# p-mc-grath/DMMFODS

Measured on AMD Instinct MI355X. Metric: training images/sec at 1280x1920 RGB+LiDAR, higher is better.
Workload: dtype f16; 1 GPU; C2 d121 early-fusion 6ch b4 1280x1920; key=c2, per_gpu_batch=4, global_batch=4, height=1280, width=1920, storage_dtype=fp16, accumulate=fp32, parallelism=dp1, weights=random-init (reference init, seed 123)

## Files before the change

dmmfods_amd/_lib.py:

```python
import ctypes as C
import os

_HERE = os.path.dirname(os.path.abspath(__file__))
LIB_PATH = os.environ.get("DMM_LIB_PATH") or os.path.join(_HERE, "libdmmfods_hip.so")

DMM_F32, DMM_F16, DMM_BF16 = 0, 1, 2
LOSS_BCE, LOSS_FOCAL = 0, 1
T_CONV, T_CONVT, T_BN_WEIGHT, T_BN_BIAS, T_BN_MEAN, T_BN_VAR, T_BN_TRACKED = range(7)
ERR_INVALID, ERR_SHAPE, ERR_HIP, ERR_STATE, ERR_NO_DEVICE = -1, -2, -3, -4, -5


class ModelDesc(C.Structure):
    _fields_ = [
        ("growth_rate", C.c_int32), ("num_blocks", C.c_int32), ("block_config", C.c_int32 * 8),
        ("num_init_features", C.c_int32), ("bn_size", C.c_int32), ("num_classes", C.c_int32),
        ("concat_before_block_num", C.c_int32), ("stream_1_in_channels", C.c_int32),
        ("stream_2_in_channels", C.c_int32), ("batch", C.c_int32), ("height", C.c_int32), ("width", C.c_int32),
        ("dtype", C.c_int32), ("loss_scale", C.c_float), ("bn_momentum", C.c_float), ("bn_eps", C.c_float),
        ("iou_threshold", C.c_float), ("use_mfma", C.c_int32),
    ]


class ConvDesc(C.Structure):
    _fields_ = [(n, C.c_int32) for n in (
# ... 119 lines not shown
    L.dmm_plan_set_encoder_frozen.argtypes = [vp, C.c_int]
    L.dmm_adam_table_bytes.argtypes = [C.c_int, i64]
    L.dmm_adam_table_bytes.restype = sz
    L.dmm_adam_table_init.argtypes = [vp, C.POINTER(AdamSegment), C.c_int, i64, C.c_int, vp]
    L.dmm_adam_step_segmented.argtypes = [vp, vp, vp, vp, i64, vp, C.c_int, C.POINTER(AdamClass), C.c_int, i64, f32, vp]
    L.dmm_adam_step_guarded_segmented.argtypes = [vp, vp, vp, vp, i64, vp, C.c_int, C.POINTER(AdamClass), C.c_int, f32, f32, f32, i32,
                                                  vp, vp, vp]
    L.dmm_adam_step_segmented_ema.argtypes = L.dmm_adam_step_segmented.argtypes + [C.POINTER(AdamEma)]
    L.dmm_adam_step_guarded_segmented_ema.argtypes = L.dmm_adam_step_guarded_segmented.argtypes + [C.POINTER(AdamEma)]
    L.dmm_grad_sumsq.argtypes = [vp, i64, i64, C.c_int, vp, vp]
    L.dmm_plan_set_dynamic_loss_scale.argtypes = [vp, vp]
    L.dmm_plan_set_grad_accumulate.argtypes = [vp, C.c_int]
    L.dmm_conv_scratch_bytes.argtypes = [C.POINTER(ConvDesc)]
    L.dmm_conv_scratch_bytes.restype = sz
    L.dmm_conv_forward.argtypes = [C.POINTER(ConvDesc), vp, vp, vp, vp, vp, vp, vp, vp]
    L.dmm_conv_logits.argtypes = [C.POINTER(ConvDesc), vp, vp, vp, vp, vp, vp, vp]
    L.dmm_conv_wgrad.argtypes = [C.POINTER(ConvDesc), vp, vp, vp, vp, vp, vp, vp]
    L.dmm_conv_dgrad.argtypes = [C.POINTER(ConvDesc), vp, vp, vp, vp, vp, vp, vp, vp, vp]
    L.dmm_conv_wgrad_ex.argtypes = [C.POINTER(ConvDesc), vp, vp, vp, vp, vp, vp, vp, C.c_int, vp, vp, vp]
    L.dmm_conv_dgrad_ex.argtypes = [C.POINTER(ConvDesc), vp, vp, vp, vp, vp, vp, vp, vp, vp, C.c_int, vp, vp, vp]
    L.dmm_conv1x1_backward_fused.argtypes = [C.POINTER(ConvDesc), vp, vp, vp, vp, vp, vp, vp, vp, vp, C.c_int, vp, vp, vp, vp]
    L.dmm_conv5_wgrad_stats.argtypes = [C.POINTER(ConvDesc), vp, vp, vp, vp, vp, vp, vp, vp, vp]
    L.dmm_plan_wgrad_batch_counts.argtypes = [vp, C.POINTER(C.c_longlong * 4)]
    L.dmm_conv_wgrad_grouped.argtypes = [C.POINTER(ConvDesc), C.c_int, vp, vp, vp, vp, vp, vp, vp, vp, vp, C.c_int, C.POINTER(C.c_int), vp]
    L.dmm_bw1_reduce_grouped.argtypes = [C.c_int, vp, vp, C.POINTER(C.c_int), C.POINTER(C.c_int), C.POINTER(C.c_int), C.c_int,
                                         C.POINTER(C.c_int), vp]
    _lib = L
    return L


EXPORTS = [
    "dmm_last_error", "dmm_version", "dmm_set_option", "dmm_plan_create", "dmm_plan_destroy", "dmm_plan_num_tensors",
    "dmm_plan_tensor_info", "dmm_plan_num_params", "dmm_plan_num_buffer_elems", "dmm_plan_workspace_bytes",
    "dmm_plan_forward_flops", "dmm_plan_bind", "dmm_plan_forward", "dmm_plan_loss_backward", "dmm_plan_backward",
    "dmm_plan_loss_metrics", "dmm_plan_num_graph_replays", "dmm_plan_set_loss", "dmm_loss_forward", "dmm_plan_num_grad_buckets", "dmm_plan_grad_bucket",
    "dmm_plan_grad_bucket_wait", "dmm_plan_profile_begin", "dmm_plan_profile_filter", "dmm_plan_profile_num_ops", "dmm_plan_profile_op",
    "dmm_plan_profile_collect", "dmm_adam_step", "dmm_conv_scratch_bytes", "dmm_conv_forward", "dmm_conv_logits", "dmm_conv_wgrad",
    "dmm_conv_dgrad", "dmm_conv_wgrad_ex", "dmm_conv_dgrad_ex", "dmm_conv1x1_backward_fused", "dmm_conv5_wgrad_stats", "dmm_last_impl", "dmm_impl_name", "dmm_impl_mask",
    "dmm_grad_guard_scratch_bytes", "dmm_guard_state_init", "dmm_adam_step_guarded", "dmm_grad_sumsq", "dmm_plan_set_dynamic_loss_scale",
    "dmm_plan_set_grad_accumulate", "dmm_plan_set_encoder_frozen",
    "dmm_adam_table_bytes", "dmm_adam_table_init", "dmm_adam_step_segmented", "dmm_adam_step_guarded_segmented",
    "dmm_adam_step_segmented_ema", "dmm_adam_step_guarded_segmented_ema",
    "dmm_plan_wgrad_batch_counts", "dmm_conv_wgrad_grouped", "dmm_bw1_reduce_grouped",
    "dmm_logit_hist_elems", "dmm_logit_hist", "dmm_augment_batch",
]
HIST_MAX_THRESHOLDS = 255


def check(rc):
    if rc == 0:
        return
    msg = lib().dmm_last_error().decode(errors="replace")
    if rc == ERR_SHAPE:
        raise ValueError(msg)
    if rc == ERR_INVALID and "fusion" in msg:
        raise AttributeError(msg)
    if rc == ERR_INVALID:
        raise ValueError(msg)
    raise DmmError(f"dmm status {rc}: {msg}")
# ... 17 lines not shown
```

dmmfods_amd/csrc/capi.cpp:

```cpp
#include <algorithm>
#include <atomic>
#include <cmath>
#include <cstdio>
#include <cstdlib>
#include <cstring>
#include <stdexcept>
#include <mutex>
#include <string>
#include <utility>
#include <vector>
#include <unistd.h>

#include "dispatch.h"
#include "plan.h"

using namespace dmm;

void plan_build_tables(dmm_plan* p);
void plan_bind(dmm_plan* p, void* ws);
void plan_size(dmm_plan* p);

static thread_local std::string g_err;
static int fail(int code, const std::string& msg) {
  g_err = msg;
// ... 210 lines not shown
    case OP_IGEMM: return launch_igemm(o.c, dt, o.epi, mfma, st, o.impl);
    case OP_WGRAD:
      if (o.impl == IMPL_WG3 && o.w.M > 0) { ++p->batch_counts[0]; ++p->batch_counts[1]; }
      return launch_wgrad(o.w, dt, mfma, st, o.impl);
    case OP_BW1: return launch_bw1(o.b1, dt, st);
    case OP_BW1RED:
      { Bw1RedGroup one; if (bw1_reduce_group_add(one, o.b1) && one.n > 0) { ++p->batch_counts[2]; ++p->batch_counts[3]; } }
      return launch_bw1_reduce(o.b1, st);
    case OP_RAWFIN: return launch_wg5_rawfin(o.rf, st);
    case OP_FIN64: return launch_wg5_fin64(o.f64, st);
    case OP_JOIN: if (o.epi == 1) lanes.join_pack(); else lanes.join_side(); return hipSuccess;
    case OP_BNFIN: return launch_bn_finalize(o.bf, st);
    case OP_BNBWD:
      if (accumulate) { BnBwdFinalizeArgs bb = o.bb; bb.accumulate = 1; return launch_bn_bwd_finalize(bb, st); }
      return launch_bn_bwd_finalize(o.bb, st);
    case OP_POOL: return launch_maxpool_fwd(o.mp, dt, st);
    case OP_POOLBWD: return launch_maxpool_bwd(o.mpb, dt, st);
    case OP_BCE: return launch_bce_metrics(o.bce, dt, st);
    case OP_PACK: return launch_pack(o.pk.descs, o.pk.prefix, o.pk.ndesc, o.pk.total_rows, dt, st, o.pk.tdescs, o.pk.tiles, o.pk.nt1, o.pk.nt9);
    case OP_APPLYCORR: return launch_apply_corr(o.ac, dt, st);
    case OP_UNPACK: return launch_unpack(o.pk.descs, o.pk.prefix, o.pk.ndesc, o.pk.total_rows, dt, o.pk.grad_scale, st, o.pk.tdescs, o.pk.tiles, o.pk.nt1, o.pk.nt9, accumulate);
    default: known = false; return hipSuccess;
  }
}

int launch_checked(dmm_plan* p, const Op& o, size_t i, hipStream_t st, Lanes& lanes, std::string& why) {
  const bool fam_check = (o.kind == OP_IGEMM || o.kind == OP_WGRAD) && o.impl != IMPL_AUTO;
  const unsigned mask_before = g_impl_mask;
  if (fam_check) g_impl_mask = 0;
  bool known = true;
  const hipError_t e = launch_record(p, o, st, lanes, known);
// ... 310 lines not shown
  if (B < 1 || NC < 1 || H < 1 || W < 1) return fail(DMM_ERR_INVALID, who + "B, NC, H and W must be >= 1");
  if ((long long)B * NC > 65535) return fail(DMM_ERR_INVALID, who + "B * NC must be <= 65535");
  if ((long long)H * W >= (1ll << 31)) return fail(DMM_ERR_INVALID, who + "H * W must be < 2^31");
  if (nthr < 1 || nthr > DMM_HIST_MAX_THRESHOLDS) return fail(DMM_ERR_INVALID, who + "nthr must be in [1, " + std::to_string(DMM_HIST_MAX_THRESHOLDS) + "]");
  for (int k = 0; k < nthr; ++k)
    if (!std::isfinite(thresholds[k])) return fail(DMM_ERR_INVALID, who + "thresholds[" + std::to_string(k) + "] is NaN or infinite");
  for (int k = 1; k < nthr; ++k)
    if (!(thresholds[k] > thresholds[k - 1])) return fail(DMM_ERR_INVALID, who + "thresholds must be strictly ascending (at index " + std::to_string(k) + ")");
  if (std::isnan(gt_threshold)) return fail(DMM_ERR_INVALID, who + "gt_threshold is NaN");
  LogitHistArgs a;
  memset(&a, 0, sizeof(a));
  a.logits = logits; a.target = target; a.counts = (unsigned long long*)counts;
  a.B = B; a.NC = NC; a.H = H; a.W = W; a.K = nthr; a.gt = gt_threshold;
  for (int k = 0; k < nthr; ++k) a.thr[k] = thresholds[k];
  HIPCHK(launch_logit_hist(a, accumulate, (hipStream_t)stream));
  return DMM_OK;
}

int dmm_augment_batch(const dmm_aug_tensor* tensors, int ntensors, const dmm_aug_sample* samples, int B, int Hs, int Ws, int Ho, int Wo,
                      const float* fill, void* stream) {
  const std::string who = "dmm_augment_batch: ";
  if (!tensors || !samples) return fail(DMM_ERR_INVALID, who + "null argument");
  if (ntensors < 1 || ntensors > DMM_AUG_MAX_TENSORS) return fail(DMM_ERR_INVALID, who + "ntensors must be in [1, " + std::to_string(DMM_AUG_MAX_TENSORS) + "]");
  if (B < 1 || Hs < 1 || Ws < 1 || Ho < 1 || Wo < 1) return fail(DMM_ERR_INVALID, who + "B, Hs, Ws, Ho and Wo must be >= 1");
  const long long splane = (long long)Hs * Ws, dplane = (long long)Ho * Wo;
  if (splane >= (1ll << 31)) return fail(DMM_ERR_INVALID, who + "Hs * Ws must be < 2^31");
  if (dplane >= (1ll << 31)) return fail(DMM_ERR_INVALID, who + "Ho * Wo must be < 2^31");
  int nch = 0;
  for (int t = 0; t < ntensors; ++t) {
    const dmm_aug_tensor& T = tensors[t];
// ... 1019 lines not shown
```

dmmfods_amd/csrc/igemm.hip:

```cpp
#include <cstdlib>
#include <type_traits>

#ifndef IGEMM_FOLD_EPI
#define IGEMM_FOLD_EPI -1
#endif
#ifndef IGEMM_FOLD_BN
#define IGEMM_FOLD_BN 0
#endif
#ifndef IGEMM_FOLD_LIN
#define IGEMM_FOLD_LIN -1
#endif
#ifndef IGEMM_FOLD_PRO
#define IGEMM_FOLD_PRO -2
#endif
#ifndef IGEMM_F32_FOLD
#define IGEMM_F32_FOLD 0
#endif
#include "common.h"
#include "dispatch.h"
#include "gather.h"
#include "isa.h"

namespace dmm {

// ... 502 lines not shown
    }
    const int nsub = a.pool2 ? 4 : 1;
    const float wgt = a.pool2 ? 0.25f : 1.f;
    for (int row = rr; row < BM && !prefetched; row += RPP) {
      const int pix = rowpix[row];
      if (pix < 0 || !colvalid) continue;
      float av[SLOT];
#pragma unroll
      for (int i = 0; i < SLOT; i += 4) {
        const f32x4 t4 = *(const f32x4*)(Cs + row * SM::STAGE_PITCH_F + cv * SLOT + i);
        av[i] = t4[0]; av[i + 1] = t4[1]; av[i + 2] = t4[2]; av[i + 3] = t4[3];
      }
      for (int sub = 0; sub < nsub; ++sub) {
        const size_t p = (size_t)pix + (sub >> 1) * a.Wout + (sub & 1);
        float xf[SLOT], gf[SLOT];
        vec_to_f32<T>(*(const V*)(bx + p * a.ldbx + n), xf);
        if (a.accumulate && g != nullptr) vec_to_f32<T>(*(const V*)(g + p * a.ldo + n), gf);
#pragma unroll
        for (int i = 0; i < SLOT; ++i) {
          const float dz = (fmaf(xf[i], sc[i], sh[i]) > 0.f) ? av[i] * wgt : 0.f;
          s1[i] += dz;
          s2[i] = fmaf(dz, (xf[i] - mu[i]) * is[i], s2[i]);
          gf[i] = (a.accumulate ? gf[i] : 0.f) + sc[i] * dz;
        }
        if (g != nullptr) *(V*)(g + p * a.ldo + n) = f32_to_vec<T>(gf);
      }
    }
  }

  constexpr bool F32FOLD = IGEMM_F32_FOLD && (IGEMM_FOLD_EPI < 0 || EPI == IGEMM_FOLD_EPI) && (IGEMM_FOLD_BN == 0 || BN == IGEMM_FOLD_BN) &&
                           (IGEMM_FOLD_LIN < 0 || (int)LIN == IGEMM_FOLD_LIN) && (IGEMM_FOLD_PRO < -1 || PRO == IGEMM_FOLD_PRO);
  if constexpr ((sizeof(T) == 4 || !MFMA) && !F32FOLD) {
// ... 152 lines not shown
```

dmmfods_amd/csrc/plan.cpp:

```cpp
#include "plan.h"

#include <algorithm>
#include <cmath>
#include <cstdio>
#include <cstdlib>
#include <cstring>
#include <map>
#include <stdexcept>

namespace dmm {

static unsigned tw1(int mt) { return 0xffffff00u | (unsigned)mt; }

std::vector<Tap> taps_conv(int R, int S, int pad) {
  std::vector<Tap> t;
  for (int ky = 0; ky < R; ++ky)
    for (int kx = 0; kx < S; ++kx) t.push_back({ky - pad, kx - pad, tw1(ky * S + kx)});
  return t;
}
std::vector<Tap> taps_conv_dgrad(int R, int S, int pad) {
  std::vector<Tap> t;
  for (int ky = 0; ky < R; ++ky)
    for (int kx = 0; kx < S; ++kx) t.push_back({pad - ky, pad - kx, tw1(ky * S + kx)});
  return t;
// ... 236 lines not shown
struct ConvRec {
  std::string wname;
  bool transposed;
  int N, Kin, R, S, pad;
  int B, Ho, Wo;
  int nseg;
  SegRec seg[2];
  int obuf, och0, ostride;
  int epi;
  bool stats;
  std::vector<PhaseRec> phases;
  int dpack[2];
  bool wgrad_transposed;
  bool shared_master;
  double flops_ref;
};
struct PoolRec { int y0buf, bn, obuf, och0; uint8_t* argmax; int C; };
struct Rec { int type; int idx; };
struct BucketRec {
  int64_t off = 0, n = 0;
  int convs_left = 0, bns_left = 0;
  int first_desc = 0, ndesc = 0, rows = 0;
  int tile0 = 0, nt1 = 0, nt9 = 0;
  int last_main = -1, last_side = -1;
};

enum LaunchRole { ROLE_STORE, ROLE_BNBWD, ROLE_LOGITS, ROLE_WGRAD , ROLE_WGRAD_T  };
const char* launch_class(int impl, LaunchRole role) {
  static const struct { LaunchRole role; int impl; const char* cls; } table[] = {
      {ROLE_STORE, IMPL_CONV3, "conv3.store"}, {ROLE_STORE, IMPL_CVP, "cvp.store"},     {ROLE_STORE, IMPL_CF, "cf.store"},
// ... 206 lines not shown
    std::string s = w;
    const char* cuts[] = {"features.", "stream_2_features.", "decoder.", "dec_out_to_heat_maps.", ".weight", "denseblock", "denselayer", "Transposed_Convolution"};
    const char* reps[] = {"f.", "s2.", "d.", "h.", "", "b", "l", "TC"};
    for (int i = 0; i < 8; ++i) {
      size_t p;
      while ((p = s.find(cuts[i])) != std::string::npos) s.replace(p, strlen(cuts[i]), reps[i]);
    }
    return s;
  }
  double conv_flops(const ConvRec& c, size_t nphases) const {
    if (c.flops_ref > 0) return c.flops_ref / (double)nphases;
    const double px = (double)c.B * c.Ho * c.Wo * (c.seg[0].mode == G_POOL2 ? 4.0 : 1.0);
    const double f = c.transposed ? 2.0 * px * c.N * c.Kin * 9.0 : 2.0 * px * c.N * c.Kin * c.R * c.S;
    return f / (double)nphases;
  }
  double src_bytes(const ConvRec& c) const {
    double b = 0;
    for (int s = 0; s < c.nseg; ++s) {
      const Buf& sb = bufs[c.seg[s].buf];
      b += (double)sb.B * sb.H * sb.W * c.seg[s].C * esz;
    }
    return b;
  }
  double out_bytes(const ConvRec& c) const {
    const Buf& ob = bufs[c.obuf];
    return (double)ob.B * ob.H * ob.W * rup(c.N, 8) * (c.epi == EPI_LOGITS ? 4 : esz);
  }
  double w_bytes(const ConvRec& c) const { return (double)c.N * c.Kin * c.R * c.S * esz; }
  const uint8_t* xat(int buf, int ch) const { return bufs[buf].x + (size_t)ch * esz; }
  uint8_t* gat(int buf, int ch) const { return bufs[buf].g ? bufs[buf].g + (size_t)ch * esz : nullptr; }

  void emit_bn_finalize(int bn) {
    Bn& b = bns[bn];
    for (auto& rg : b.ranges) {
// ... 40 lines not shown
      const Op& po = (*ops)[first + ph];
      copy_phase(merged, po, ph);
      merged.flops += po.flops; merged.bytes += po.bytes;
    }
    if (!accept(merged)) return;
    ops->resize(first);
    ops->push_back(merged);
  }
  static void copy_fwd_phase(ConvArgs& m, const ConvArgs& po, int ph, int ntaps0) {
    m.nphase = 4;
    for (int t = 0; t < 4; ++t) m.ph_taps0[ph][t] = po.seg[0].taps[t < ntaps0 ? t : 0];
    m.ph_wpack[ph] = po.wpack;
    m.ph_py[ph] = (signed char)po.py; m.ph_px[ph] = (signed char)po.px;
  }

  void emit_conv_fwd(ConvRec& c) {
    for (int s = 0; s < c.nseg; ++s) {
      const int bn = c.seg[s].bn;
      if (bn < 0 || (s == 1 && bn == c.seg[0].bn)) continue;
      emit_bn_finalize(bn);
    }
    const Buf& ob = bufs[c.obuf];
    const bool mfma = d.use_mfma != 0;
    for (auto& ph : c.phases) {
      Op& o = push(OP_IGEMM);
      o.epi = c.epi;
      ConvArgs& a = o.c;
      a.nseg = c.nseg;
      for (int s = 0; s < c.nseg; ++s) fill_fwd_seg(a.seg[s], c.seg[s], (s == 1 && !ph.taps1.empty()) ? ph.taps1 : ph.taps);
      a.B = c.B; a.Ho = c.Ho; a.Wo = c.Wo; a.M = c.B * c.Ho * c.Wo;
      const PackDesc& pd = P.packs[ph.pack];
      a.wpack = pd.dst;
      a.N = c.N; a.Npad = pd.Npad;
      a.out = (void*)xat(c.obuf, c.och0);
      a.ldo = ob.ld; a.Hout = ob.H; a.Wout = ob.W;
      a.ostride = c.ostride; a.py = ph.py; a.px = ph.px;
      if (c.stats && ob.ssum) { a.stat_sum = ob.ssum + c.och0; a.stat_sq = ob.ssq + c.och0; a.stat_stride = ob.ld; }
      const double np = (double)c.phases.size();
      o.impl = igemm_pick(a, dtype, c.epi, mfma, deny);
      tag(o, ncls(o.impl, c.epi == EPI_LOGITS ? ROLE_LOGITS : ROLE_STORE, pd.Npad), short_name(c.wname), conv_flops(c, c.phases.size()),
          (src_bytes(c) + out_bytes(c)) / np + w_bytes(c) / np);
      if (c.epi == EPI_LOGITS) {
        if (training) P.logits_op_train = (int)ops->size() - 1; else P.logits_op_eval = (int)ops->size() - 1;
      }
// ... 152 lines not shown
    if (st.eff_compact != nullptr && o.impl == IMPL_WG3 && !leaf_scope) {
      st.wg3_op = o;
      ops->pop_back();
      st.wg3_held = true;
    } else if (st.r1_sbuf != nullptr && o.impl == IMPL_WG5 && !leaf_scope && c.seg[0].bn >= 0) {
      st.r1_idx = (int)ops->size() - 1;
    }
  }

  void emit_wgrad_phases(ConvRec& c, int wseg) {
    const int Nst = rup(c.N, 8);
    for (auto& ph : c.phases) {
      Op& o = push(OP_WGRAD);
      WgradArgs& a = o.w;
      a.nseg = wseg;
      for (int s = 0; s < wseg; ++s) fill_fwd_seg(a.seg[s], c.seg[s], (s == 1 && !ph.taps1.empty()) ? ph.taps1 : ph.taps);
      a.B = c.B; a.Ho = c.Ho; a.Wo = c.Wo; a.M = c.B * c.Ho * c.Wo;
      fill_grad_seg(a.dy, c.obuf, c.och0, Nst, taps_conv(1, 1, 0), c.ostride);
      one_tap_seg(a.dy, ph.py, ph.px);
      const PackDesc& pd = P.packs[ph.pack];
      a.N = c.N; a.Npad = pd.Npad;
      a.dpack = (float*)pd.dpack;
      const double np = (double)c.phases.size();
      o.impl = wgrad_pick(a, dtype, d.use_mfma != 0, deny);
      tag(o, ncls(o.impl, ROLE_WGRAD, pd.Npad), short_name(c.wname), conv_flops(c, c.phases.size()) * (wseg < c.nseg ? (double)c.seg[0].Cw / c.Kin : 1.0),
          (src_bytes(c) + grad_reads(c) * out_bytes(c)) / np + w_bytes(c) * 4.0 / esz / np);
    }
    if (c.phases.size() == 4 && wseg == 1 && !P.sw.no_wgp_merge)
      merge_last_four_phases(
          [](const Op& po, const Op& f) {
            const int nt = po.w.seg[0].ntaps;
// ... 245 lines not shown
    a.mean = bns[p.bn].mean; a.invstd = bns[p.bn].invstd;
    a.red1 = bns[p.bn].red1; a.red2 = bns[p.bn].red2; a.stat_stride = bns[p.bn].cp;
    tag(o, "maxpool.bwd", "pool0", 0, (2.0 * yb.B * yb.H * yb.W + 2.0 * ob.B * ob.H * ob.W) * p.C * esz + (double)ob.B * ob.H * ob.W * p.C);
    yb.ginit = true;
    emit_bn_bwd_finalize(p.bn);
  }

  ConvRec& new_conv(const std::string& wname, bool transposed, int N, int Kin, int R, int S, int pad) {
    ConvRec c;
    c.wname = wname; c.transposed = transposed; c.N = N; c.Kin = Kin; c.R = R; c.S = S; c.pad = pad;
    c.nseg = 1; c.ostride = 1; c.epi = EPI_STORE; c.stats = true;
    c.dpack[0] = c.dpack[1] = -1;
    c.wgrad_transposed = false;
    c.shared_master = false;
    c.flops_ref = 0;
    memset(c.seg, 0, sizeof(c.seg));
    c.seg[0].bn = c.seg[1].bn = -1;
    convs.push_back(c);
    recs.push_back({0, (int)convs.size() - 1});
    return convs.back();
  }
  void finish_conv(ConvRec& c) {
    for (auto& ph : c.phases) ph.pack = add_pack(c, ph.taps, false, 0, &ph.taps1);
    for (int s = 0; s < c.nseg; ++s) {
      if (c.seg[s].dgrad != DG_NONE) c.dpack[s] = add_pack(c, dgrad_taps(c, c.seg[s].dgrad), true, s);
    }
    if (c.nseg == 1 && !c.transposed && c.seg[0].mode == G_PLAIN && c.seg[0].istride == 1 && c.seg[0].dgrad == DG_FLIP &&
        c.R * c.S > 1 && rup(c.N, 8) < c.seg[0].C && c.phases.size() == 1) {
      c.wgrad_transposed = true;
      PackDesc& dp = P.packs[c.dpack[0]];
// ... 42 lines not shown
      static const int matz_k = lab_int("DMM_MATZ_DENSE_K", 1 << 30);
      const int y1 = new_buf(X.B, X.H, X.W, rup(bw, 8), true, true, K >= matz_k);
      const int n1 = new_bn(q + ".norm1", K);
      bn_range(n1, xb, base, 0, K);
      plain_conv(q + ".conv1.weight", bw, K, 1, 0, xb, base, G_PLAIN, 1, n1, DG_FLIP, X.H, X.W, y1, 0);
      const int n2 = new_bn(q + ".norm2", bw);
      bn_range(n2, y1, 0, 0, bw);
      plain_conv(q + ".conv2.weight", g.k, bw, 3, 1, y1, 0, G_PLAIN, 1, n2, DG_FLIP, X.H, X.W, xb, base + K);
    }
  }

  void transition(const std::string& p, int xb, int base, int C, int obuf, int och0) {
    const Buf X = bufs[xb];
    const int n = new_bn(p + ".norm", C);
    bn_range(n, xb, base, 0, C);
    plain_conv(p + ".conv.weight", C / 2, C, 1, 0, xb, base, G_POOL2, 1, n, DG_POOL2, X.H / 2, X.W / 2, obuf, och0);
  }

  void build() {
    const int B = d.batch, H = d.height, Wd = d.width;
    if (H % 32 || Wd % 32 || H <= 0 || Wd <= 0) throw std::domain_error("spatial size must be a multiple of 32");
    if (g.k % 8 || g.nif % 8 || (g.bs * g.k) % 8) throw std::invalid_argument("channel counts must be multiples of 8");
    if (g.s1 + g.s2 > 8 || g.s1 < 1) throw std::invalid_argument("at most 8 raw input channels are supported");
    for (int b = 0; b + 1 < g.nb; ++b)
      if (g.cout[b] % 16) throw std::invalid_argument("block widths must be multiples of 16");
    if (g.nc > 8) throw std::invalid_argument("num_classes > 8 unsupported");

    in1 = new_buf(B, H, Wd, 8, g.fusion != 2, true);
    if (g.fusion == 2) { in2 = new_buf(B, H, Wd, 8, false, false); inH = new_buf(B, H, Wd, 8, true, true); }
    else inH = in1;

// ... 405 lines not shown
PlanSwitches PlanSwitches::from_environment() {
  PlanSwitches s;
  auto on = [](const char* n) { const char* v = getenv(n); return v != nullptr && !(v[0] == '0' && v[1] == 0); };
  s.no_pack_tiles = on("DMM_NO_PACK_TILES");
  s.no_hf = on("DMM_NO_HF");
  s.no_c3_merge = on("DMM_NO_C3_MERGE");
  s.no_cvp_merge = on("DMM_NO_CVP_MERGE");
  s.no_wgp_merge = on("DMM_NO_WGP_MERGE");
  s.no_two_pass = on("DMM_NO_TWO_PASS");
  s.no_eff_compact = on("DMM_NO_EFF_COMPACT");
  s.no_s2_interleave = on("DMM_NO_S2_INTERLEAVE");
  s.no_raw_stats = on("DMM_NO_RAW_STATS");
  s.no_r1_stats = on("DMM_NO_R1_STATS");
  const char* pc = getenv("DMM_PACK_CUT");
  s.pack_cut = pc ? std::max(1, atoi(pc)) : 0;
  return s;
}

void plan_size(dmm_plan* p) {
  p->packs.clear();
  Builder b(*p, true, nullptr);
  b.build();
  b.emit_all();
  p->zero_bytes = (b.Z.off + 255) / 256 * 256;
  p->zero_bwd_bytes = (b.ZB.off + 255) / 256 * 256;
  p->main_bytes = (b.W.off + 255) / 256 * 256;
  p->fwd_flops = b.flops;
  p->packs.clear();
}

// ... 37 lines not shown
```

dmmfods_amd/csrc/plan.h:

```cpp
#pragma once
#include <cstring>
#include <stdexcept>
#include <string>
#include <vector>

#include "../../include/dmmfods_hip.h"
#include "common.h"
#include "pointwise.h"

namespace dmm {

struct plan_sizing_error : std::runtime_error { using std::runtime_error::runtime_error; };

struct TensorInfo {
  std::string name;
  int kind, ndim;
  int64_t shape[4];
  int64_t off;
};

struct Tap {
  int dy, dx;
  unsigned tapw;
};
// ... 56 lines not shown
bool flushes_batches(const Op& o);
Lane route(const Op& o, bool overlap, bool forked, bool batch_main);

}

struct GradBucket {
  int64_t off = 0, n = 0;
  int ev_main = -1, ev_side = -1;
  int ready = -1;
};

struct PlanSwitches {
  bool no_pack_tiles = false, no_hf = false, no_c3_merge = false, no_cvp_merge = false, no_wgp_merge = false, no_two_pass = false,
       no_eff_compact = false, no_s2_interleave = false, no_raw_stats = false, no_r1_stats = false;
  int pack_cut = 0;
  static PlanSwitches from_environment();
};

struct dmm_plan {
  dmm_model_desc desc;
  PlanSwitches sw;
  unsigned deny = 0;
  std::vector<dmm::TensorInfo> tensors;
  int64_t nparams = 0, nbuf = 0;
  size_t zero_bytes = 0, zero_bwd_bytes = 0, main_bytes = 0;
  double fwd_flops = 0;
  bool bound = false;
  void* ws = nullptr;
  float *params = nullptr, *grads = nullptr, *buffers = nullptr;
  std::vector<dmm::Op> fwd_train, fwd_eval, bwd;
// ... 39 lines not shown
```

dmmfods_amd/csrc/pointwise.h:

```cpp
#pragma once
#include "../../include/dmmfods_hip.h"
#include "common.h"

namespace dmm {

struct ConvertArgs {
  const float* src1;
  const float* src2;
  int C1, C2;
  void* dst;
  int B, H, W;
  double* stat_sum;
  double* stat_sq;
  float scale;
  const float* dyn_scale;
};

struct BnFinalizeArgs {
  const double* sum;
  const double* sq;
  int stat_stride;
  double count;
  double count_unbiased;
  const float* gamma;
// ... 29 lines not shown
  int C;
  int accumulate;
};

struct MaxpoolArgs {
  const void* y0;
  int ld0, H0, W0, B, C;
  const float* scale;
  const float* shift;
  void* out;
  int ldo, Hp, Wp;
  unsigned char* argmax;
  double* stat_sum;
  double* stat_sq;
  int stat_stride;
};

struct MaxpoolBwdArgs {
  const void* y0;
  int ld0, H0, W0, B, C;
  const float* scale;
  const float* shift;
  const void* gpool;
  const void* xpool;
  const float* q;
  const float* r;
  const float* ql;
  const float* rl;
  const float* mean;
  const float* invstd;
  int ldg, Hp, Wp;
// ... 153 lines not shown
  alignas(16) unsigned char block[4096];
};
bool wg3_group_add(Wg3Group& G, const WgradArgs& a, int dtype);
hipError_t wg3_group_launch(Wg3Group& G, hipStream_t st);
hipError_t launch_igemm(const ConvArgs& a, int dtype, int epi, bool mfma, hipStream_t st, int impl = IMPL_AUTO, unsigned deny = 0);
hipError_t launch_wgrad(WgradArgs a, int dtype, bool mfma, hipStream_t st, int impl = IMPL_AUTO, unsigned deny = 0);
int igemm_pick(const ConvArgs& a, int dtype, int epi, bool mfma, unsigned deny);
int wgrad_pick(const WgradArgs& a, int dtype, bool mfma, unsigned deny);
hipError_t launch_wg5_rawfin(const RawFinArgs& a, hipStream_t st);
hipError_t launch_wg5_fin64(const Fin64Args& a, hipStream_t st);
hipError_t launch_convert_input(const ConvertArgs& a, int dtype, hipStream_t st);
hipError_t launch_bn_finalize(const BnFinalizeArgs& a, hipStream_t st);
hipError_t launch_bn_bwd_finalize(const BnBwdFinalizeArgs& a, hipStream_t st);
hipError_t launch_maxpool_fwd(const MaxpoolArgs& a, int dtype, hipStream_t st);
hipError_t launch_maxpool_bwd(const MaxpoolBwdArgs& a, int dtype, hipStream_t st);
hipError_t launch_bce_metrics(const BceArgs& a, int dtype, hipStream_t st);
hipError_t launch_logit_hist(const LogitHistArgs& a, int accumulate, hipStream_t st);
int logit_hist_grid_x(int planes, size_t plane);
hipError_t launch_logit_hist(const LogitHistArgs& a, int accumulate, hipStream_t st);
int logit_hist_grid_x(int planes, size_t plane);
hipError_t launch_augment(const AugArgs& a, int nchannels, int nsamples, hipStream_t st);
unsigned augment_grid_x(int Ho, int Wo);
hipError_t launch_grad_sumsq(const GradSumsqArgs& a, hipStream_t st);
hipError_t launch_guard_finalize(const GuardFinalizeArgs& a, hipStream_t st);
hipError_t launch_adam_segmented(const AdamSegArgs& a, hipStream_t st);
hipError_t launch_guard_init(dmm_guard_state* dev, float scale, int64_t applied, int32_t tracker, hipStream_t st);
hipError_t launch_apply_corr(const ApplyCorrArgs& a, int dtype, hipStream_t st);
hipError_t launch_pack(const PackDesc* descs_dev, const int* prefix_dev, int ndesc, int total_rows, int dtype, hipStream_t st,
                       const PackDesc* tile_descs = nullptr, const PackTile* tiles_dev = nullptr, int nt1 = 0, int nt9 = 0);
hipError_t launch_unpack(const PackDesc* descs_dev, const int* prefix_dev, int ndesc, int total_rows, int dtype, float grad_scale,
// ... 69 lines not shown
```

dmmfods_amd/csrc/pointwise.hip:

```cpp
#include <type_traits>

#include "common.h"
#include "gather.h"
#include "pointwise.h"

namespace dmm {

thread_local int g_last_impl = IMPL_AUTO;
thread_local unsigned g_impl_mask = 0;

template <typename T>
__global__ __launch_bounds__(256) void convert_input_kernel(ConvertArgs a) {
  __shared__ double red[16];
  if (threadIdx.x < 16) red[threadIdx.x] = 0.0;
  __syncthreads();
  const size_t plane = (size_t)a.H * a.W;
  const size_t npix = (size_t)a.B * plane;
  double s1[8], s2[8];
#pragma unroll
  for (int c = 0; c < 8; ++c) { s1[c] = 0.0; s2[c] = 0.0; }
  const float scale = a.dyn_scale != nullptr ? a.scale * *a.dyn_scale : a.scale;
  for (size_t p = (size_t)blockIdx.x * blockDim.x + threadIdx.x; p < npix; p += (size_t)gridDim.x * blockDim.x) {
    const size_t b = p / plane, rem = p - b * plane;
    float v[8];
// ... 136 lines not shown
    }
  }
  block_channel_reduce<SLOT>(red, a.C, c, s1, s2, a.stat_sum, a.stat_sq, a.stat_stride);
}

hipError_t launch_maxpool_fwd(const MaxpoolArgs& a, int dtype, hipStream_t st) {
  const int slot = dtype == DT_F32 ? 4 : 8;
  const int rpb = 256 / (a.C / slot);
  const int npix = a.B * a.Hp * a.Wp;
  int grid = (npix + rpb - 1) / rpb;
  if (grid > 2048) grid = 2048;
  const size_t smem = 2 * a.C * sizeof(double);
  if (dtype == DT_F16) hipLaunchKernelGGL(maxpool_fwd_kernel<f16>, dim3(grid), dim3(256), smem, st, a);
  else if (dtype == DT_BF16) hipLaunchKernelGGL(maxpool_fwd_kernel<bf16>, dim3(grid), dim3(256), smem, st, a);
  else hipLaunchKernelGGL(maxpool_fwd_kernel<float>, dim3(grid), dim3(256), smem, st, a);
  return hipGetLastError();
}

template <typename T>
__global__ __launch_bounds__(256) void maxpool_bwd_kernel(MaxpoolBwdArgs a) {
  constexpr int SLOT = TT<T>::SLOT;
  typedef typename TT<T>::vec V;
  extern __shared__ double red[];
  for (int i = threadIdx.x; i < 2 * a.C; i += blockDim.x) red[i] = 0.0;
  __syncthreads();
  const int ncv = a.C / SLOT;
  const int cv = threadIdx.x % ncv, rl = threadIdx.x / ncv, rpb = blockDim.x / ncv;
  const int c = cv * SLOT;
  float sc[SLOT], sh[SLOT], q[SLOT], rr[SLOT], qlo[SLOT], rlo[SLOT];
  double s1[SLOT], s2[SLOT];
// ... 557 lines not shown
```

dmmfods_amd/csrc/wgrad.hip:

```cpp
#include <algorithm>
#include <cstdlib>
#include <type_traits>

#include "common.h"
#include "dispatch.h"
#include "gather.h"
#include "isa.h"

namespace dmm {

#ifndef WGRAD_DIST_HEAVY
#define WGRAD_DIST_HEAVY 1
#endif
#ifndef WGRAD_DBG
#define WGRAD_DBG 0
#endif
constexpr int KW = 128;

template <typename T> struct WgCfg;
template <> struct WgCfg<f16> { static constexpr int BMW = 64; };
template <> struct WgCfg<bf16> { static constexpr int BMW = 64; };
template <> struct WgCfg<float> { static constexpr int BMW = 32; };

template <typename T, int WBN>
// ... 299 lines not shown
static hipError_t launch_w(const WgradArgs& a, bool mfma, hipStream_t st) {
  typedef WgradSmem<T, WBN> SM;
  const int ntiles = a.Npad / WBN;
  const int splits = (a.M + a.rows_per_split - 1) / a.rows_per_split;
  int pq = seg_pro(a.seg[0]);
  for (int s = 1; s < a.nseg; ++s) if (seg_pro(a.seg[s]) != pq) pq = -1;
  const int pp = seg_pro(a.dy);
  const bool lin = a.nseg == 1 && seg_lin(a.seg[0], a) && seg_lin(a.dy, a);
  LdsLauncher<WgradArgs> run;
  if (!mfma) {
    if constexpr (std::is_same<T, bf16>::value) return hipErrorNotSupported;
    else run = launch_lds<wgrad_kernel<T, WBN, false, -1, -1, false, WDIST(WBN, -1, -1)>, WgradArgs>;
  }
  else if (lin && pp == 2 && pq == 1) run = launch_lds<wgrad_kernel<T, WBN, true, 2, 1, true, WDIST(WBN, 2, 1)>, WgradArgs>;
  else if (lin && pp == 0 && pq == 1) run = launch_lds<wgrad_kernel<T, WBN, true, 0, 1, true, WDIST(WBN, 0, 1)>, WgradArgs>;
  else if (pp == 0 && pq == 1) run = launch_lds<wgrad_kernel<T, WBN, true, 0, 1, false, WDIST(WBN, 0, 1)>, WgradArgs>;
  else if (pp == 2 && pq == 1) run = launch_lds<wgrad_kernel<T, WBN, true, 2, 1, false, WDIST(WBN, 2, 1)>, WgradArgs>;
  else if (pp == 1 && pq == 2) run = launch_lds<wgrad_kernel<T, WBN, true, 1, 2, false, WDIST(WBN, 1, 2)>, WgradArgs>;
  else if (pp == 2 && pq == 0) run = launch_lds<wgrad_kernel<T, WBN, true, 2, 0, false, WDIST(WBN, 2, 0)>, WgradArgs>;
  else if (pp == 1 && pq == 0) run = launch_lds<wgrad_kernel<T, WBN, true, 1, 0, false, WDIST(WBN, 1, 0)>, WgradArgs>;
  else run = launch_lds<wgrad_kernel<T, WBN, true, -1, -1, false, WDIST(WBN, -1, -1)>, WgradArgs>;
  return run(SM::bytes > 48 * 1024 ? SM::bytes : 0, ntiles * a.kgroups * splits, NTHREADS, SM::bytes, st, a);
}

template <typename T>
hipError_t launch_wt(const WgradArgs& a, bool mfma, hipStream_t st) {
  if (a.Npad % 128 == 0) return launch_w<T, 128>(a, mfma, st);
  if (a.Npad % 64 == 0) return launch_w<T, 64>(a, mfma, st);
  return launch_w<T, 32>(a, mfma, st);
}
// ... 78 lines not shown
```

include/dmmfods_hip.h:

```cpp
#ifndef DMMFODS_HIP_H
#define DMMFODS_HIP_H
#include <stddef.h>
#include <stdint.h>

#ifdef __cplusplus
extern "C" {
#endif

typedef enum {
  DMM_OK = 0,
  DMM_ERR_INVALID = -1,
  DMM_ERR_SHAPE = -2,
  DMM_ERR_HIP = -3,
  DMM_ERR_STATE = -4,
  DMM_ERR_NO_DEVICE = -5
} dmm_status;

enum { DMM_F32 = 0, DMM_F16 = 1, DMM_BF16 = 2 };

enum { DMM_T_CONV = 0, DMM_T_CONVT = 1, DMM_T_BN_WEIGHT = 2, DMM_T_BN_BIAS = 3, DMM_T_BN_MEAN = 4, DMM_T_BN_VAR = 5,
       DMM_T_BN_TRACKED = 6 };

typedef struct {
  int32_t growth_rate;
// ... 150 lines not shown
int dmm_plan_set_dynamic_loss_scale(dmm_plan* plan, const float* scale_dev);

typedef struct {
  int32_t dtype, use_mfma;
  int32_t B, H, W;
  int32_t Cin, Cout;
  int32_t R, S, stride, pad;
  int32_t transposed;
  int32_t mode;
  int32_t bn_relu;
} dmm_conv_desc;

size_t dmm_conv_scratch_bytes(const dmm_conv_desc* d);
int dmm_conv_forward(const dmm_conv_desc* d, const void* x, const float* w, const float* scale, const float* shift, void* y,
                     double* stats, void* scratch, void* stream);
int dmm_conv_logits(const dmm_conv_desc* d, const void* x, const float* w, const float* scale, const float* shift, float* logits,
                    void* scratch, void* stream);
int dmm_conv_wgrad(const dmm_conv_desc* d, const void* x, const void* dy, const float* scale, const float* shift, float* dw,
                   void* scratch, void* stream);
int dmm_conv_dgrad(const dmm_conv_desc* d, const void* x, const void* dy, const float* w, const float* scale, const float* shift,
                   void* gx, double* red, void* scratch, void* stream);


int dmm_conv_wgrad_ex(const dmm_conv_desc* d, const void* x, const void* dy, const float* scale, const float* shift, const void* yfwd,
                      const float* q, const float* r, int transposed_form, float* dw, void* scratch, void* stream);
int dmm_conv_dgrad_ex(const dmm_conv_desc* d, const void* x, const void* dy, const float* w, const float* scale, const float* shift,
                      const void* yfwd, const float* q, const float* r, void* gx, int accumulate, double* red, void* scratch,
                      void* stream);
int dmm_conv5_wgrad_stats(const dmm_conv_desc* d, const void* x, const void* dy, const float* w, const float* scale, const float* shift,
                          float* dw, double* red, void* scratch, void* stream);
// ... 19 lines not shown
```

Measured before the change: 166.7 img/s.

## Precompute pooled BN-ReLU transition input once for large transition convs

For DenseNet transition layers whose pooled output has enough rows, the BN+ReLU+2x2 average pool is now materialized once into a new buffer by a dedicated kernel. The forward 1x1 conv and its wgrad then read that plain buffer instead of redoing the pool-gather with BN/ReLU inside every GEMM tile. This trades extra memory and one pointwise pass for less redundant gather work in the conv kernels. It also adds wgrad kernel instantiations for the new operand pattern, debug switches in igemm, and a standalone C API entry.

```diff
diff --git a/dmmfods_amd/_lib.py b/dmmfods_amd/_lib.py
--- a/dmmfods_amd/_lib.py
+++ b/dmmfods_amd/_lib.py
@@ -157,6 +157,7 @@
     L.dmm_conv_scratch_bytes.argtypes = [C.POINTER(ConvDesc)]
     L.dmm_conv_scratch_bytes.restype = sz
     L.dmm_conv_forward.argtypes = [C.POINTER(ConvDesc), vp, vp, vp, vp, vp, vp, vp, vp]
+    L.dmm_pool_act.argtypes = [C.c_int, vp, C.c_int, C.c_int, C.c_int, C.c_int, C.c_int, vp, vp, vp, C.c_int, vp]
     L.dmm_conv_logits.argtypes = [C.POINTER(ConvDesc), vp, vp, vp, vp, vp, vp, vp]
     L.dmm_conv_wgrad.argtypes = [C.POINTER(ConvDesc), vp, vp, vp, vp, vp, vp, vp]
     L.dmm_conv_dgrad.argtypes = [C.POINTER(ConvDesc), vp, vp, vp, vp, vp, vp, vp, vp, vp]
@@ -185,7 +186,7 @@
     "dmm_adam_table_bytes", "dmm_adam_table_init", "dmm_adam_step_segmented", "dmm_adam_step_guarded_segmented",
     "dmm_adam_step_segmented_ema", "dmm_adam_step_guarded_segmented_ema",
     "dmm_plan_wgrad_batch_counts", "dmm_conv_wgrad_grouped", "dmm_bw1_reduce_grouped",
-    "dmm_logit_hist_elems", "dmm_logit_hist", "dmm_augment_batch",
+    "dmm_logit_hist_elems", "dmm_logit_hist", "dmm_augment_batch", "dmm_pool_act",
 ]
 HIST_MAX_THRESHOLDS = 255
 
diff --git a/dmmfods_amd/csrc/capi.cpp b/dmmfods_amd/csrc/capi.cpp
--- a/dmmfods_amd/csrc/capi.cpp
+++ b/dmmfods_amd/csrc/capi.cpp
@@ -248,7 +248,7 @@
     case OP_BNBWD:
       if (accumulate) { BnBwdFinalizeArgs bb = o.bb; bb.accumulate = 1; return launch_bn_bwd_finalize(bb, st); }
       return launch_bn_bwd_finalize(o.bb, st);
-    case OP_POOL: return launch_maxpool_fwd(o.mp, dt, st);
+    case OP_POOL: return launch_pool(o.mp, dt, st);
     case OP_POOLBWD: return launch_maxpool_bwd(o.mpb, dt, st);
     case OP_BCE: return launch_bce_metrics(o.bce, dt, st);
     case OP_PACK: return launch_pack(o.pk.descs, o.pk.prefix, o.pk.ndesc, o.pk.total_rows, dt, st, o.pk.tdescs, o.pk.tiles, o.pk.nt1, o.pk.nt9);
@@ -589,6 +589,29 @@
   a.B = B; a.NC = NC; a.H = H; a.W = W; a.K = nthr; a.gt = gt_threshold;
   for (int k = 0; k < nthr; ++k) a.thr[k] = thresholds[k];
   HIPCHK(launch_logit_hist(a, accumulate, (hipStream_t)stream));
+  return DMM_OK;
+}
+
+int dmm_pool_act(int dtype, const void* x, int B, int H, int W, int C, int ldx, const float* scale, const float* shift, void* out, int ldo,
+                 void* stream) {
+  const std::string who = "dmm_pool_act: ";
+  if (!x || !scale || !shift || !out) return fail(DMM_ERR_INVALID, who + "null argument");
+  if (dtype != DMM_F32 && dtype != DMM_F16 && dtype != DMM_BF16) return fail(DMM_ERR_INVALID, who + "unknown dtype");
+  const int slot = dtype == DMM_F32 ? 4 : 8;
+  if (B < 1 || H < 2 || W < 2) return fail(DMM_ERR_INVALID, who + "B must be >= 1, H and W >= 2");
+  if (H % 2 || W % 2) return fail(DMM_ERR_INVALID, who + "H and W must be even (2x2 windows, stride 2)");
+  if ((long long)B * (H / 2) * (W / 2) >= (1ll << 31)) return fail(DMM_ERR_INVALID, who + "B * H/2 * W/2 must be < 2^31");
+  if (C < slot || C % slot) return fail(DMM_ERR_INVALID, who + "C must be a positive multiple of the 16-byte slot (" + std::to_string(slot) + " channels)");
+  if (ldx < C || ldo < C || ldx % slot || ldo % slot) return fail(DMM_ERR_INVALID, who + "pitches must be multiples of the slot and >= C");
+  if ((uintptr_t)x % 16 || (uintptr_t)out % 16 || (uintptr_t)scale % 16 || (uintptr_t)shift % 16)
+    return fail(DMM_ERR_INVALID, who + "x, out, scale and shift must be 16-byte aligned");
+  MaxpoolArgs a;
+  memset(&a, 0, sizeof(a));
+  a.mode = POOL_ACT2;
+  a.y0 = x; a.ld0 = ldx; a.H0 = H; a.W0 = W; a.B = B; a.C = C;
+  a.scale = scale; a.shift = shift;
+  a.out = out; a.ldo = ldo; a.Hp = H / 2; a.Wp = W / 2;
+  HIPCHK(launch_pool(a, dtype, (hipStream_t)stream));
   return DMM_OK;
 }
 
diff --git a/dmmfods_amd/csrc/igemm.hip b/dmmfods_amd/csrc/igemm.hip
--- a/dmmfods_amd/csrc/igemm.hip
+++ b/dmmfods_amd/csrc/igemm.hip
@@ -540,8 +540,14 @@
       for (int sub = 0; sub < nsub; ++sub) {
         const size_t p = (size_t)pix + (sub >> 1) * a.Wout + (sub & 1);
         float xf[SLOT], gf[SLOT];
-        vec_to_f32<T>(*(const V*)(bx + p * a.ldbx + n), xf);
-        if (a.accumulate && g != nullptr) vec_to_f32<T>(*(const V*)(g + p * a.ldo + n), gf);
+        const size_t pl = (IGEMM_DBG & 64) ? (size_t)pix : p;
+        if (IGEMM_DBG & 128) {
+#pragma unroll
+          for (int i = 0; i < SLOT; ++i) { xf[i] = 1.f; gf[i] = 0.f; }
+        } else {
+          vec_to_f32<T>(*(const V*)(bx + pl * a.ldbx + n), xf);
+          if (a.accumulate && g != nullptr) vec_to_f32<T>(*(const V*)(g + pl * a.ldo + n), gf);
+        }
 #pragma unroll
         for (int i = 0; i < SLOT; ++i) {
           const float dz = (fmaf(xf[i], sc[i], sh[i]) > 0.f) ? av[i] * wgt : 0.f;
diff --git a/dmmfods_amd/csrc/plan.cpp b/dmmfods_amd/csrc/plan.cpp
--- a/dmmfods_amd/csrc/plan.cpp
+++ b/dmmfods_amd/csrc/plan.cpp
@@ -274,6 +274,7 @@
   bool wgrad_transposed;
   bool shared_master;
   double flops_ref;
+  int abuf;
 };
 struct PoolRec { int y0buf, bn, obuf, och0; uint8_t* argmax; int C; };
 struct Rec { int type; int idx; };
@@ -510,10 +511,15 @@
     const double f = c.transposed ? 2.0 * px * c.N * c.Kin * 9.0 : 2.0 * px * c.N * c.Kin * c.R * c.S;
     return f / (double)nphases;
   }
+  SegRec operand_seg(const ConvRec& c, int s) const {
+    SegRec sr = c.seg[s];
+    if (s == 0 && c.abuf >= 0) { sr.buf = c.abuf; sr.ch0 = 0; sr.mode = G_PLAIN; sr.istride = 1; sr.bn = -1; sr.bn_c0 = 0; }
+    return sr;
+  }
   double src_bytes(const ConvRec& c) const {
     double b = 0;
     for (int s = 0; s < c.nseg; ++s) {
-      const Buf& sb = bufs[c.seg[s].buf];
+      const Buf& sb = bufs[operand_seg(c, s).buf];
       b += (double)sb.B * sb.H * sb.W * c.seg[s].C * esz;
     }
     return b;
@@ -584,12 +590,28 @@
     m.ph_py[ph] = (signed char)po.py; m.ph_px[ph] = (signed char)po.px;
   }
 
+  void emit_pool_act(const ConvRec& c) {
+    const SegRec& sr = c.seg[0];
+    const Buf &sb = bufs[sr.buf], &ab = bufs[c.abuf];
+    Op& o = push(OP_POOL);
+    MaxpoolArgs& a = o.mp;
+    a.mode = POOL_ACT2;
+    a.y0 = xat(sr.buf, sr.ch0); a.ld0 = sb.ld; a.H0 = sb.H; a.W0 = sb.W; a.B = sb.B; a.C = sr.C;
+    a.scale = bns[sr.bn].scale + sr.bn_c0; a.shift = bns[sr.bn].shift + sr.bn_c0;
+    a.out = ab.x; a.ldo = ab.ld; a.Hp = ab.H; a.Wp = ab.W;
+    std::string layer = short_name(c.wname);
+    if (layer.size() > 5 && layer.compare(layer.size() - 5, 5, ".conv") == 0) layer.replace(layer.size() - 5, 5, ".norm");
+    const double npix_in = (double)sb.B * sb.H * sb.W;
+    tag(o, "poolact", layer, 0, npix_in * sr.C * esz + npix_in / 4 * sr.C * esz);
+  }
+
   void emit_conv_fwd(ConvRec& c) {
     for (int s = 0; s < c.nseg; ++s) {
       const int bn = c.seg[s].bn;
       if (bn < 0 || (s == 1 && bn == c.seg[0].bn)) continue;
       emit_bn_finalize(bn);
     }
+    if (c.abuf >= 0) emit_pool_act(c);
     const Buf& ob = bufs[c.obuf];
     const bool mfma = d.use_mfma != 0;
     for (auto& ph : c.phases) {
@@ -597,7 +619,7 @@
       o.epi = c.epi;
       ConvArgs& a = o.c;
       a.nseg = c.nseg;
-      for (int s = 0; s < c.nseg; ++s) fill_fwd_seg(a.seg[s], c.seg[s], (s == 1 && !ph.taps1.empty()) ? ph.taps1 : ph.taps);
+      for (int s = 0; s < c.nseg; ++s) fill_fwd_seg(a.seg[s], operand_seg(c, s), (s == 1 && !ph.taps1.empty()) ? ph.taps1 : ph.taps);
       a.B = c.B; a.Ho = c.Ho; a.Wo = c.Wo; a.M = c.B * c.Ho * c.Wo;
       const PackDesc& pd = P.packs[ph.pack];
       a.wpack = pd.dst;
@@ -780,7 +802,7 @@
       Op& o = push(OP_WGRAD);
       WgradArgs& a = o.w;
       a.nseg = wseg;
-      for (int s = 0; s < wseg; ++s) fill_fwd_seg(a.seg[s], c.seg[s], (s == 1 && !ph.taps1.empty()) ? ph.taps1 : ph.taps);
+      for (int s = 0; s < wseg; ++s) fill_fwd_seg(a.seg[s], operand_seg(c, s), (s == 1 && !ph.taps1.empty()) ? ph.taps1 : ph.taps);
       a.B = c.B; a.Ho = c.Ho; a.Wo = c.Wo; a.M = c.B * c.Ho * c.Wo;
       fill_grad_seg(a.dy, c.obuf, c.och0, Nst, taps_conv(1, 1, 0), c.ostride);
       one_tap_seg(a.dy, ph.py, ph.px);
@@ -1056,6 +1078,7 @@
     c.wgrad_transposed = false;
     c.shared_master = false;
     c.flops_ref = 0;
+    c.abuf = -1;
     memset(c.seg, 0, sizeof(c.seg));
     c.seg[0].bn = c.seg[1].bn = -1;
     convs.push_back(c);
@@ -1128,7 +1151,10 @@
     const Buf X = bufs[xb];
     const int n = new_bn(p + ".norm", C);
     bn_range(n, xb, base, 0, C);
+    int abuf = -1;
+    if ((long long)X.B * (X.H / 2) * (X.W / 2) >= P.sw.pool_once_rows) abuf = new_buf(X.B, X.H / 2, X.W / 2, C, false, false);
     plain_conv(p + ".conv.weight", C / 2, C, 1, 0, xb, base, G_POOL2, 1, n, DG_POOL2, X.H / 2, X.W / 2, obuf, och0);
+    convs.back().abuf = abuf;
   }
 
   void build() {
@@ -1564,6 +1590,7 @@
   s.no_r1_stats = on("DMM_NO_R1_STATS");
   const char* pc = getenv("DMM_PACK_CUT");
   s.pack_cut = pc ? std::max(1, atoi(pc)) : 0;
+  if (const char* po = getenv("DMM_POOL_ONCE_ROWS")) s.pool_once_rows = std::max(0ll, atoll(po));
   return s;
 }
 
diff --git a/dmmfods_amd/csrc/plan.h b/dmmfods_amd/csrc/plan.h
--- a/dmmfods_amd/csrc/plan.h
+++ b/dmmfods_amd/csrc/plan.h
@@ -94,6 +94,8 @@
   bool no_pack_tiles = false, no_hf = false, no_c3_merge = false, no_cvp_merge = false, no_wgp_merge = false, no_two_pass = false,
        no_eff_compact = false, no_s2_interleave = false, no_raw_stats = false, no_r1_stats = false;
   int pack_cut = 0;
+  static constexpr long long POOL_ONCE_ROWS_DEFAULT = 512;
+  long long pool_once_rows = POOL_ONCE_ROWS_DEFAULT;
   static PlanSwitches from_environment();
 };
 
diff --git a/dmmfods_amd/csrc/pointwise.h b/dmmfods_amd/csrc/pointwise.h
--- a/dmmfods_amd/csrc/pointwise.h
+++ b/dmmfods_amd/csrc/pointwise.h
@@ -67,7 +67,9 @@
   double* stat_sum;
   double* stat_sq;
   int stat_stride;
-};
+  int mode;
+};
+enum PoolMode { POOL_MAX3 = 0, POOL_ACT2 = 1 };
 
 struct MaxpoolBwdArgs {
   const void* y0;
@@ -251,6 +253,10 @@
 hipError_t launch_bn_bwd_finalize(const BnBwdFinalizeArgs& a, hipStream_t st);
 hipError_t launch_maxpool_fwd(const MaxpoolArgs& a, int dtype, hipStream_t st);
 hipError_t launch_maxpool_bwd(const MaxpoolBwdArgs& a, int dtype, hipStream_t st);
+hipError_t launch_pool_act(const MaxpoolArgs& a, int dtype, hipStream_t st);
+inline hipError_t launch_pool(const MaxpoolArgs& a, int dtype, hipStream_t st) {
+  return a.mode == POOL_ACT2 ? launch_pool_act(a, dtype, st) : launch_maxpool_fwd(a, dtype, st);
+}
 hipError_t launch_bce_metrics(const BceArgs& a, int dtype, hipStream_t st);
 hipError_t launch_logit_hist(const LogitHistArgs& a, int accumulate, hipStream_t st);
 int logit_hist_grid_x(int planes, size_t plane);
diff --git a/dmmfods_amd/csrc/pointwise.hip b/dmmfods_amd/csrc/pointwise.hip
--- a/dmmfods_amd/csrc/pointwise.hip
+++ b/dmmfods_amd/csrc/pointwise.hip
@@ -174,6 +174,55 @@
   if (dtype == DT_F16) hipLaunchKernelGGL(maxpool_fwd_kernel<f16>, dim3(grid), dim3(256), smem, st, a);
   else if (dtype == DT_BF16) hipLaunchKernelGGL(maxpool_fwd_kernel<bf16>, dim3(grid), dim3(256), smem, st, a);
   else hipLaunchKernelGGL(maxpool_fwd_kernel<float>, dim3(grid), dim3(256), smem, st, a);
+  return hipGetLastError();
+}
+
+template <typename T>
+__global__ __launch_bounds__(256) void pool_act_kernel(MaxpoolArgs a) {
+  constexpr int SLOT = TT<T>::SLOT;
+  typedef typename TT<T>::vec V;
+  const int ncv = a.C / SLOT;
+  const size_t total = (size_t)a.B * a.Hp * a.Wp * ncv;
+  const T* y0 = (const T*)a.y0;
+  T* out = (T*)a.out;
+  for (size_t i = (size_t)blockIdx.x * blockDim.x + threadIdx.x; i < total; i += (size_t)gridDim.x * blockDim.x) {
+    const size_t p = i / ncv;
+    const int c = (int)(i - p * ncv) * SLOT;
+    int b, oy, ox;
+    row_to_byx((int)p, a.Hp, a.Wp, b, oy, ox);
+    V win[4];
+#pragma unroll
+    for (int k = 0; k < 4; ++k)
+      win[k] = *(const V*)(y0 + ((size_t)(b * a.H0 + 2 * oy + (k >> 1)) * a.W0 + (2 * ox + (k & 1))) * a.ld0 + c);
+    float sc[SLOT], sh[SLOT], acc[SLOT];
+    load_f32s<SLOT>(a.scale + c, sc);
+    load_f32s<SLOT>(a.shift + c, sh);
+#pragma unroll
+    for (int j = 0; j < SLOT; ++j) acc[j] = 0.f;
+#pragma unroll
+    for (int k = 0; k < 4; ++k) {
+      float f[SLOT];
+      vec_to_f32<T>(win[k], f);
+#pragma unroll
+      for (int j = 0; j < SLOT; ++j) acc[j] += fmaxf(fmaf(f[j], sc[j], sh[j]), 0.f);
+    }
+#pragma unroll
+    for (int j = 0; j < SLOT; ++j) acc[j] *= 0.25f;
+    *(V*)(out + p * a.ldo + c) = f32_to_vec<T>(acc);
+  }
+}
+
+hipError_t launch_pool_act(const MaxpoolArgs& a, int dtype, hipStream_t st) {
+  const int slot = dtype == DT_F32 ? 4 : 8;
+  if (a.B <= 0 || a.Hp <= 0 || a.Wp <= 0 || a.H0 != 2 * a.Hp || a.W0 != 2 * a.Wp || a.C <= 0 || a.C % slot || a.ld0 % slot || a.ldo % slot ||
+      a.ld0 < a.C || a.ldo < a.C || (long long)a.B * a.Hp * a.Wp > 0x7fffffffLL)
+    return hipErrorInvalidValue;
+  const size_t total = (size_t)a.B * a.Hp * a.Wp * (a.C / slot);
+  size_t grid = (total + 255) / 256;
+  if (grid > 4096) grid = 4096;
+  if (dtype == DT_F16) hipLaunchKernelGGL(pool_act_kernel<f16>, dim3((unsigned)grid), dim3(256), 0, st, a);
+  else if (dtype == DT_BF16) hipLaunchKernelGGL(pool_act_kernel<bf16>, dim3((unsigned)grid), dim3(256), 0, st, a);
+  else hipLaunchKernelGGL(pool_act_kernel<float>, dim3((unsigned)grid), dim3(256), 0, st, a);
   return hipGetLastError();
 }
 
diff --git a/dmmfods_amd/csrc/wgrad.hip b/dmmfods_amd/csrc/wgrad.hip
--- a/dmmfods_amd/csrc/wgrad.hip
+++ b/dmmfods_amd/csrc/wgrad.hip
@@ -337,6 +337,8 @@
   }
   else if (lin && pp == 2 && pq == 1) run = launch_lds<wgrad_kernel<T, WBN, true, 2, 1, true, WDIST(WBN, 2, 1)>, WgradArgs>;
   else if (lin && pp == 0 && pq == 1) run = launch_lds<wgrad_kernel<T, WBN, true, 0, 1, true, WDIST(WBN, 0, 1)>, WgradArgs>;
+  else if (lin && pp == 2 && pq == 0) run = launch_lds<wgrad_kernel<T, WBN, true, 2, 0, true, WDIST(WBN, 2, 0)>, WgradArgs>;
+  else if (lin && pp == 0 && pq == 0) run = launch_lds<wgrad_kernel<T, WBN, true, 0, 0, true, WDIST(WBN, 0, 0)>, WgradArgs>;
   else if (pp == 0 && pq == 1) run = launch_lds<wgrad_kernel<T, WBN, true, 0, 1, false, WDIST(WBN, 0, 1)>, WgradArgs>;
   else if (pp == 2 && pq == 1) run = launch_lds<wgrad_kernel<T, WBN, true, 2, 1, false, WDIST(WBN, 2, 1)>, WgradArgs>;
   else if (pp == 1 && pq == 2) run = launch_lds<wgrad_kernel<T, WBN, true, 1, 2, false, WDIST(WBN, 1, 2)>, WgradArgs>;
diff --git a/include/dmmfods_hip.h b/include/dmmfods_hip.h
--- a/include/dmmfods_hip.h
+++ b/include/dmmfods_hip.h
@@ -188,6 +188,8 @@
 size_t dmm_conv_scratch_bytes(const dmm_conv_desc* d);
 int dmm_conv_forward(const dmm_conv_desc* d, const void* x, const float* w, const float* scale, const float* shift, void* y,
                      double* stats, void* scratch, void* stream);
+int dmm_pool_act(int dtype, const void* x, int B, int H, int W, int C, int ldx, const float* scale, const float* shift, void* out, int ldo,
+                 void* stream);
 int dmm_conv_logits(const dmm_conv_desc* d, const void* x, const float* w, const float* scale, const float* shift, float* logits,
                     void* scratch, void* stream);
 int dmm_conv_wgrad(const dmm_conv_desc* d, const void* x, const void* dy, const float* scale, const float* shift, float* dw,
```

Result: no change. 166.5 img/s (-0.1%).
